# happyjin/Gaussian_process

Hardware: AMD Instinct MI355X
Metric: GP-fit+predict sec and achieved fp64 TFLOP/s, N=65536 d=8, 1/2/4/8 MI355X (higher is better)
Workload: dtype f64; 1 GPU; GP fit+predict N=65536 d=8 n_test=4096 (BASELINE configs[2]); N=65536, d=8, n_test=4096, partition=single GPU

## Files before the change

### gaussian_process_amd/csrc/dev_api.hip

```cpp
#include "gpmi_ctx.h"

using namespace gpmi;

extern "C" {

int gpmi_dev_rbf_rows(void* stream, const double* X_dev, int64_t N, int64_t d, int64_t row0,
                      int64_t nrows, int64_t ncols, double sigma, double ell, double noise_var,
                      double* out_dev, int64_t ld) {
    if (!X_dev || !out_dev) return fail_arg("gpmi_dev_rbf_rows: null pointer");
    if (nrows % TILE || ncols % TILE || row0 % TILE || ld < ncols || ld % 2)
        return fail_arg("gpmi_dev_rbf_rows: sizes must be multiples of 128");
    RbfArgs r;
    r.A = r.B = X_dev; r.nA = r.nB = N; r.d = d; r.row0 = row0; r.nrows = nrows; r.ncols = ncols;
    r.coef = -.5 * (1 / (ell * ell)); r.sig2 = sigma * sigma; r.diag_add = noise_var; r.symmetric = 1;
    r.out = out_dev; r.ld = ld;
    HIP_TRY(launch_rbf((hipStream_t)stream, r));
    return GPMI_OK;
}

int gpmi_dev_rbf_cross(void* stream, const double* Xs_dev, int64_t n, const double* X_dev, int64_t N,
                       int64_t d, int64_t row0, int64_t nrows, int64_t ncols, double sigma, double ell,
                       double* out_dev, int64_t ld) {
    if (!Xs_dev || !X_dev || !out_dev) return fail_arg("gpmi_dev_rbf_cross: null pointer");
    if (nrows % TILE || ncols % TILE || ld < ncols || ld % 2)
// ... 48 lines not shown
                       int64_t ncols, double* out_dev, int64_t ld) {
    if (!Xs_dev || !Xcols_dev || !out_dev) return fail_arg("gpmi_dev_cov_cross: null pointer");
    if (nrows % TILE || ncols % TILE || ld < ncols || ld % 2 || col0 < 0)
        return fail_arg("gpmi_dev_cov_cross: sizes must be multiples of 128");
    RbfArgs r;
    r.A = Xs_dev; r.B = Xcols_dev; r.nA = n; r.nB = ncols_real > 0 ? ncols_real : 0; r.d = d; r.row0 = 0; r.nrows = nrows; r.ncols = ncols;
    const int rc = dev_cov_args(r, kind, params, nparams, "gpmi_dev_cov_cross");
    if (rc) return rc;
    r.diag_add = 0.; r.symmetric = 0; r.delta_square = square ? 1 : 0; r.delta_col0 = col0;
    r.out = out_dev; r.ld = ld;
    HIP_TRY(launch_rbf((hipStream_t)stream, r));
    return GPMI_OK;
}

int gpmi_dev_potrf_block(void* stream, double* A_dev, int64_t ld, int64_t nb, int64_t col_offset,
                         int64_t* info_dev) {
    if (!A_dev || !info_dev) return fail_arg("gpmi_dev_potrf_block: null pointer");
    if (nb <= 0 || nb % TILE || ld % 2) return fail_arg("gpmi_dev_potrf_block: nb must be a multiple of 128");
    HIP_TRY(panel_factor((hipStream_t)stream, A_dev, ld, nb, nb, col_offset, info_dev));
    return GPMI_OK;
}

int gpmi_dev_trsm_block(void* stream, const double* L_dev, int64_t ldl, double* X_dev, int64_t ldx,
                        int64_t m, int64_t nb) {
    if (!L_dev || !X_dev) return fail_arg("gpmi_dev_trsm_block: null pointer");
    if (m < 0 || m % TILE || nb <= 0 || nb % IB || ldl % 2 || ldx % 2)
        return fail_arg("gpmi_dev_trsm_block: m must be a multiple of 128, nb of 64");
    if (m == 0) return GPMI_OK;
    HIP_TRY(trsm_block((hipStream_t)stream, L_dev, ldl, X_dev, ldx, m, nb));
    return GPMI_OK;
}

int gpmi_dev_border_sweep(void* stream, const double* L_dev, int64_t ldl, int64_t ncols, double* X_dev, int64_t ldx,
                          int64_t rows) {
    if (!L_dev || !X_dev) return fail_arg("gpmi_dev_border_sweep: null pointer");
    if (rows < 1 || rows > 16) return fail_arg("gpmi_dev_border_sweep: rows must be in 1..16");
    if (ncols < 0 || ncols % TILE) return fail_arg("gpmi_dev_border_sweep: ncols must be a multiple of 128");
    if (ldl % 2 || ldx % 2 || ldl < ncols || ldx < ncols)
        return fail_arg("gpmi_dev_border_sweep: ldl and ldx must be even and at least ncols");
    if ((reinterpret_cast<uintptr_t>(L_dev) & 15) || (reinterpret_cast<uintptr_t>(X_dev) & 15))
        return fail_arg("gpmi_dev_border_sweep: both pointers must be 16-byte aligned");
    HIP_TRY(launch_border_sweep((hipStream_t)stream, L_dev, ldl, ncols, X_dev, ldx, rows));
    return GPMI_OK;
}

int gpmi_dev_gemm_nt(void* stream, double* C_dev, int64_t ldc, const double* A_dev, int64_t lda,
                     const double* B_dev, int64_t ldb, int64_t M, int64_t N, int64_t K, int lower,
                     int64_t diag_off) {
    if (!C_dev || !A_dev || !B_dev) return fail_arg("gpmi_dev_gemm_nt: null pointer");
    if (M < 0 || N < 0 || K < 0 || M % TILE || N % IB || K % 16 || ldc % 2 || lda % 2 || ldb % 2)
        return fail_arg("gpmi_dev_gemm_nt: M%128, N%64, K%16 must be 0");
    GemmArgs g = gemm_minus(C_dev, ldc, A_dev, lda, B_dev, ldb, M, N, K);
    g.lower = lower; g.diag_off = diag_off;
    HIP_TRY(launch_gemm_nt((hipStream_t)stream, g));
    return GPMI_OK;
}

int gpmi_dev_gemm_nt_rowmap(void* stream, double* C_dev, int64_t ldc, const double* A_dev, int64_t lda,
                            const double* B_dev, int64_t ldb, int64_t M, int64_t N, int64_t K,
                            const int32_t* row_ncols_dev, int64_t row_block_rows) {
    if (!C_dev || !A_dev || !B_dev || !row_ncols_dev) return fail_arg("gpmi_dev_gemm_nt_rowmap: null pointer");
    if (M < 0 || N < 0 || K < 0 || M % TILE || N % IB || K % 16 || ldc % 2 || lda % 2 || ldb % 2 ||
        row_block_rows <= 0 || row_block_rows % TILE)
        return fail_arg("gpmi_dev_gemm_nt_rowmap: M%128, N%64, K%16, row_block_rows%128 must be 0");
    GemmArgs g = gemm_minus(C_dev, ldc, A_dev, lda, B_dev, ldb, M, N, K);
    g.row_ncols = row_ncols_dev; g.row_block_tiles = (int)(row_block_rows / TILE);
    HIP_TRY(launch_gemm_nt((hipStream_t)stream, g));
    return GPMI_OK;
}

int gpmi_dev_gemm_nt_rowmap_host(void* stream, double* C_dev, int64_t ldc, const double* A_dev, int64_t lda,
                                 const double* B_dev, int64_t ldb, int64_t M, int64_t N, int64_t K,
                                 const int32_t* row_ncols_dev, const int32_t* row_ncols_host, int64_t row_bands,
                                 int64_t row_block_rows) {
    if (!C_dev || !A_dev || !B_dev || !row_ncols_dev || !row_ncols_host) return fail_arg("gpmi_dev_gemm_nt_rowmap_host: null pointer");
    if (M < 0 || N < 0 || K < 0 || M % TILE || N % IB || K % 16 || ldc % 2 || lda % 2 || ldb % 2 ||
        row_block_rows <= 0 || row_block_rows % TILE || row_bands * row_block_rows < M)
        return fail_arg("gpmi_dev_gemm_nt_rowmap_host: M%128, N%64, K%16, row_block_rows%128 must be 0 and the map must cover M");
    GemmArgs g = gemm_minus(C_dev, ldc, A_dev, lda, B_dev, ldb, M, N, K);
    g.row_ncols = row_ncols_dev; g.row_block_tiles = (int)(row_block_rows / TILE);
    g.row_ncols_host = row_ncols_host; g.row_bands = (int)row_bands;
    HIP_TRY(launch_gemm_nt((hipStream_t)stream, g));
    return GPMI_OK;
}

int gpmi_dev_gemm_nt_blocks(void* stream, double* C_dev, int64_t ldc, const double* A_dev, int64_t lda,
                            const double* B_dev, int64_t ldb, const int64_t* b_block_off_dev, int64_t b_block_rows,
                            int64_t M, int64_t N, int64_t K, const int32_t* row_ncols_dev,
                            const int32_t* row_ncols_host, int64_t row_bands, int64_t row_block_rows) {
    if (!C_dev || !A_dev || !B_dev || !b_block_off_dev) return fail_arg("gpmi_dev_gemm_nt_blocks: null pointer");
    if (M < 0 || N < 0 || K < 0 || M % TILE || N % TILE || K % 16 || K < 32 || ldc % 2 || lda % 2 || ldb % 2 ||
        b_block_rows <= 0 || b_block_rows % TILE)
        return fail_arg("gpmi_dev_gemm_nt_blocks: M%128, N%128, K%16 (K >= 32), b_block_rows%128 must be 0");
    if ((row_ncols_dev != nullptr) != (row_ncols_host != nullptr))
        return fail_arg("gpmi_dev_gemm_nt_blocks: the row map needs both its device and its host copy");
    if (row_ncols_dev && (row_block_rows <= 0 || row_block_rows % TILE || row_bands * row_block_rows < M))
        return fail_arg("gpmi_dev_gemm_nt_blocks: row_block_rows%128 must be 0 and the map must cover M");
    GemmArgs g = gemm_minus(C_dev, ldc, A_dev, lda, B_dev, ldb, M, N, K);
    g.b_block_off = b_block_off_dev; g.b_block_rows = b_block_rows;
    if (row_ncols_dev) {
        g.row_ncols = row_ncols_dev; g.row_block_tiles = (int)(row_block_rows / TILE);
        g.row_ncols_host = row_ncols_host; g.row_bands = (int)row_bands;
    }
    HIP_TRY(launch_gemm_nt((hipStream_t)stream, g));
    return GPMI_OK;
}
// ... 104 lines not shown
```

### gaussian_process_amd/csrc/driver.hip

```cpp
#include "gpmi_ctx.h"
#include "gpmi_plan.h"

namespace gpmi {

hipError_t panel_rec(hipStream_t s, double* A, int64_t ld, int64_t mrows, int64_t off, int64_t w,
                     int64_t col_offset, int64_t* info) {
    hipError_t e;
    const bool fused = tuning().panel_fused && w % 128 == 0 && off % 128 == 0;
    const int64_t leaf = fused ? 128 : IB;
    if (w <= leaf) {
        double* Ajj = A + off * ld + off;
        const int64_t below = mrows - off - leaf;
        if (fused) {
            if ((e = launch_potrf128(s, Ajj, ld, col_offset + off, info)) != hipSuccess) return e;
            if (below > 0) return launch_trsm128(s, Ajj, ld, A + (off + leaf) * ld + off, ld, below);
            return hipSuccess;
        }
        if ((e = launch_potf2_64(s, Ajj, ld, col_offset + off, info)) != hipSuccess) return e;
        if (below > 0) return launch_trsm_rlt64(s, Ajj, ld, A + (off + IB) * ld + off, ld, below);
        return hipSuccess;
    }
    const int64_t h = (w / 2) / leaf * leaf;
    if ((e = panel_rec(s, A, ld, mrows, off, h, col_offset, info)) != hipSuccess) return e;
    {
        const int64_t c0 = off + h;
        const int64_t r0 = c0 / TILE * TILE;
        const GemmArgs g = gemm_minus_lower(A + r0 * ld + c0, ld, A + r0 * ld + off, ld, A + c0 * ld + off, ld, mrows - r0,
                                            w - h, h, r0 - c0);
        if ((e = launch_gemm_nt(s, g)) != hipSuccess) return e;
    }
    return panel_rec(s, A, ld, mrows, off + h, w - h, col_offset, info);
}

hipError_t panel_factor(hipStream_t s, double* A, int64_t ld, int64_t nb, int64_t mrows,
                        int64_t col_offset, int64_t* info) {
    return panel_rec(s, A, ld, mrows, 0, nb, col_offset, info);
}

hipError_t trsm_rec(hipStream_t s, const double* L, int64_t ldl, double* X, int64_t ldx, int64_t m,
                    int64_t off, int64_t w) {
    hipError_t e;
    const bool fused = tuning().panel_fused && w % 128 == 0 && off % 128 == 0 && m % 128 == 0;
    const int64_t leaf = fused ? 128 : IB;
    if (w <= leaf) {
        if (fused) return launch_trsm128(s, L + off * ldl + off, ldl, X + off, ldx, m);
        return launch_trsm_rlt64(s, L + off * ldl + off, ldl, X + off, ldx, m);
    }
    const int64_t h = (w / 2) / leaf * leaf;
    if ((e = trsm_rec(s, L, ldl, X, ldx, m, off, h)) != hipSuccess) return e;
    const GemmArgs g = gemm_minus(X + off + h, ldx, X + off, ldx, L + (off + h) * ldl + off, ldl, m, w - h, h);
    if ((e = launch_gemm_nt(s, g)) != hipSuccess) return e;
    return trsm_rec(s, L, ldl, X, ldx, m, off + h, w - h);
}

hipError_t trsm_block(hipStream_t s, const double* L, int64_t ldl, double* X, int64_t ldx,
                      int64_t m, int64_t nb) {
    return trsm_rec(s, L, ldl, X, ldx, m, 0, nb);
}

hipError_t cholesky_inplace(gpmi_ctx* c, double* A, int64_t ld, int64_t ncols, int64_t nrows,
                            int64_t* info, bool account, int64_t carried_rows) {
    hipError_t e;
    hipStream_t sm = c->stream;
    const int64_t NB = c->block(ncols);
    const bool la = c->lookahead_for(ncols);
    hipStream_t sp_ = la ? c->pstream : sm;
    const bool slack = la && ncols >= 49152;
    SharingScope shallow(la ? Sharing::beside_update().with_panel_slack(slack) : sharing());
    const int slot_p = account ? GPMI_T_CHOL_PANEL : GPMI_T_COUNT - 1;
    const int slot_t = account ? GPMI_T_CHOL_TRAIL : GPMI_T_COUNT - 1;
    if (la && (e = c->order(sm, sp_)) != hipSuccess) return e;
    auto trail = [&](hipStream_t st, bool counted, int64_t r0, int64_t c0, int64_t k, int64_t nb, int64_t ncol_upd) -> hipError_t {
        GemmArgs g = gemm_minus_lower(A + r0 * ld + c0, ld, A + r0 * ld + k, ld, A + c0 * ld + k, ld, nrows - r0, ncol_upd,
                                      nb, r0 - c0);
        g.role = counted ? 1 : 0;
        const GemmRoute route = gemm_nt_route(g);
        const bool dma = gemm_kernel_is_dma(route.kernel);
        size_t sp = c->span_begin(counted ? (dma ? slot_t : GPMI_T_COUNT - 1) : slot_p, st);
        hipError_t er = launch_gemm_nt(st, g, route);
        c->span_end(sp, st);
        if (account && dma && counted) {
            c->stage_ms[GPMI_T_TRAIL_LAUNCHES] += 1.0;
            c->stage_ms[GPMI_T_TRAIL_FLOPS] += gemm_nt_algorithmic_flops(g, ncols - r0 + 1 + carried_rows);
        }
        return er;
    };
    hipEvent_t ev_b = nullptr;
    for (int64_t k = 0; k < ncols; k += NB) {
        const int64_t nb = std::min<int64_t>(NB, ncols - k);
        size_t sp = c->span_begin(slot_p, sp_);
        {
            SharingScope panel_forms(!la ? sharing().large_lds()
                                     : (ncols - k >= c->shallow_min ? Sharing::beside_update() : Sharing::chip_shared_only()).with_panel_slack(slack));
            e = panel_factor(sp_, A + k * ld + k, ld, nb, nrows - k, k, info);
        }
        c->span_end(sp, sp_);
        if (e != hipSuccess) return e;
        if (la && (e = c->order(sp_, sm)) != hipSuccess) return e;
        const int64_t r0 = k + nb;
        if (r0 >= ncols) continue;
        if (!la) {
            if ((e = trail(sm, true, r0, r0, k, nb, ncols - r0)) != hipSuccess) return e;
            continue;
        }
        const int64_t nbn = std::min<int64_t>(NB, ncols - r0);
        if (ev_b && (e = hipStreamWaitEvent(sp_, ev_b, 0)) != hipSuccess) return e;
        if ((e = trail(sp_, false, r0, r0, k, nb, nbn)) != hipSuccess) return e;
        if (r0 + nbn < ncols) {
            if ((e = trail(sm, true, r0 + nbn, r0 + nbn, k, nb, ncols - r0 - nbn)) != hipSuccess) return e;
            ev_b = c->new_event();
            if (!ev_b) return c->ev_error;
            if ((e = hipEventRecord(ev_b, sm)) != hipSuccess) return e;
        }
    }
    return hipSuccess;
}

RbfArgs rbf_cross(const gpmi_ctx* c, const double* A, int64_t nA, const Box& ba, const double* B, int64_t nB, const Box& bb,
                  int64_t row0, int64_t nrows, int64_t ncols, double* out, int64_t ld) {
    RbfArgs r;
    r.A = A; r.B = B;
    r.nA = nA; r.nB = nB; r.d = c->d; r.row0 = row0; r.nrows = nrows; r.ncols = ncols;
    r.coef = c->coef; r.sig2 = c->sig2;
    r.kind = c->kind; r.kp0 = c->kp0; r.kp1 = c->kp1;
    for (int i = 0; i < 11; ++i) r.kpv[i] = c->kpv[i];
    r.diag_add = 0.; r.symmetric = 0;
    r.delta_square = (A == c->x_test() && B == c->x_train() && nA == nB) ? 1 : 0;
    r.max_sq = box_max_sq(ba, bb);
// ... 202 lines not shown
```

### gaussian_process_amd/csrc/gemm_dma.hip

```cpp
#include <algorithm>
#include <cstdlib>
#include <type_traits>

#include "gpmi_internal.h"
#include "gpmi_plan.h"
#include <atomic>
#include <mutex>

namespace gpmi {

typedef double d4 __attribute__((ext_vector_type(4)));
typedef double d2 __attribute__((ext_vector_type(2)));

#define GPMI_LDS __attribute__((address_space(3)))
#define GPMI_GLB __attribute__((address_space(1)))
#define GPMI_CONST __attribute__((address_space(4)))

struct GemmDmaDev {
    double* C;
    const double* A;
    const double* B;
    int64_t ldc, lda, ldb;
    int Tm, Tn;
    int nchunks;
    int lower;
    int64_t diag_off;
    const int32_t* row_ncols;
    int row_block_tiles;
    const int64_t* b_block_off;
    int b_block_tiles;
    int S, logS, SM, SN, tri, nsuper;
    int pair;
    int sprefix[DMA_MAX_SM + 1];
    unsigned long long* stamps;
    int dbg;
    struct PersistSlot* slot;
    int nblocks;
};

struct PersistSlot {
    unsigned ctr[8];
    unsigned done;
    unsigned pad[7];
};

template <class PT>
__device__ __forceinline__ bool dma_block_to_tile(const PT& p, int b, int& ti, int& tj) {
    return plan_block_to_tile(p, b, ti, tj);
}

__device__ __forceinline__ bool dma_map_tile(const GemmDmaDev& p, int& ti, int& tj) {
    return dma_block_to_tile(p, blockIdx.x, ti, tj);
}

constexpr int DMA_TM = PLAN_TILE, DMA_TN = PLAN_TILE;
template <class PT>
__device__ __forceinline__ bool dma_tile_live(const PT& p, int ti, int tj) {
    return plan_tile_live(p, ti, tj, p.row_ncols);
}
constexpr int DMA_STAGE_SLOTS = (DMA_TM + DMA_TN) * 8;
constexpr int DMA_STAGES = 3;

constexpr unsigned TICKET_NONE = 0xFFFFFFFFu;

template <class PT>
__device__ __forceinline__ unsigned ticket_draw(const PT& p, int xcd) {
    const unsigned per = (unsigned)p.nblocks >> 3;
#pragma unroll 1
    for (int t = 0; t < 8; ++t) {
        const int x = (xcd + t) & 7;
        if (t && __hip_atomic_load(&p.slot->ctr[x], __ATOMIC_RELAXED, __HIP_MEMORY_SCOPE_AGENT) >= per) continue;
        const unsigned w = atomicAdd(&p.slot->ctr[x], 1u);
        if (w < per) return w * 8u + (unsigned)x;
    }
    return TICKET_NONE;
}

template <int MI, bool DBG, bool TICKET = false>
__device__ __forceinline__ void gemm_nt_dma_body(const GemmDmaDev& p) {
    constexpr int NWAVES = 16 / MI;
    constexpr int DPW = 32 / NWAVES;
    constexpr int RPW = DMA_TM / NWAVES;
    constexpr int NFR = MI + 4;
    const int dbg = DBG ? p.dbg : 0;
    extern __shared__ __attribute__((aligned(16))) char smem_raw[];
    const int tid = threadIdx.x;
    volatile GPMI_LDS int* mbox = (volatile GPMI_LDS int*)(smem_raw + DMA_STAGES * DMA_STAGE_SLOTS * 16);
    unsigned blk = blockIdx.x, nxt_blk = TICKET_NONE;
    int par = 0;
    if constexpr (TICKET) {
        if (tid == 0) mbox[0] = (int)ticket_draw(p, (int)(blockIdx.x & 7));
        __syncthreads();
        blk = (unsigned)__builtin_amdgcn_readfirstlane(mbox[0]);
        par = 1;
    }
  for (;;) {
    int ti = 0, tj = 0;
    bool live;
    if constexpr (TICKET) {
        if (blk == TICKET_NONE) break;
// ... 793 lines not shown
hipError_t launch_gemm_nt_small(hipStream_t s, const GemmArgs& a, const GemmRoute& r) {
    GemmSmallDev p;
    p.C = a.C; p.A = a.A; p.B = a.B; p.ldc = a.ldc; p.lda = a.lda; p.ldb = a.ldb;
    p.Tm = (int)(a.M / SM_T); p.Tn = (int)(a.N / SM_T); p.nchunks = (int)(a.K / 16);
    p.lower = a.lower; p.diag_off = a.diag_off;
    static PerDeviceOnce once;
    const hipError_t ea = once.run([&]() -> hipError_t {
        return hipFuncSetAttribute((const void*)gemm_nt_small_kernel<8>, hipFuncAttributeMaxDynamicSharedMemorySize, (int)(8 * GEMM_SMALL_STAGE));
    });
    if (ea != hipSuccess) return ea;
    if (r.kernel == GemmKernel::Small3) hipLaunchKernelGGL(gemm_nt_small_kernel<3>, dim3(r.grid), dim3(256), r.lds, s, p);
    else hipLaunchKernelGGL(gemm_nt_small_kernel<8>, dim3(r.grid), dim3(256), r.lds, s, p);
    return hipGetLastError();
}

struct PersistPool {
    static constexpr int SLOTS = 16384;
    PersistSlot* base = nullptr;
    int groups = 0;
    std::atomic<unsigned> head{0};
    PersistSlot* next() { return base + (head.fetch_add(1, std::memory_order_relaxed) % SLOTS); }
};

static PersistPool* persist_pool() {
    static std::mutex mu;
    static PersistPool pools[16];
    int dev = 0;
    if (hipGetDevice(&dev) != hipSuccess || dev < 0 || dev >= 16) return nullptr;
    PersistPool& pl = pools[dev];
    std::lock_guard<std::mutex> lock(mu);
    if (!pl.base) {
        hipDeviceProp_t prop;
        if (hipGetDeviceProperties(&prop, dev) != hipSuccess) return nullptr;
        void* q = nullptr;
        if (hipMalloc(&q, sizeof(PersistSlot) * PersistPool::SLOTS) != hipSuccess) return nullptr;
        if (hipMemset(q, 0, sizeof(PersistSlot) * PersistPool::SLOTS) != hipSuccess) { (void)hipFree(q); return nullptr; }
        pl.groups = (prop.multiProcessorCount / 8) * 8;
        if (pl.groups < 8) { (void)hipFree(q); return nullptr; }
        const void* fns[] = {(const void*)gemm_nt_dma_persist_kernel, (const void*)chol_trailing_update_persist_kernel,
                             (const void*)gemm_nt_dma_ticket_kernel, (const void*)chol_trailing_update_ticket_kernel};
        for (const void* f : fns)
            if (hipFuncSetAttribute(f, hipFuncAttributeMaxDynamicSharedMemorySize,
                                    (int)(DMA_STAGES * DMA_STAGE_SLOTS * 16 + 16)) != hipSuccess) { (void)hipFree(q); return nullptr; }
        pl.base = static_cast<PersistSlot*>(q);
    }
    return &pl;
}

int gemm_resident_groups() {
    const PersistPool* pool = persist_pool();
    return pool ? pool->groups : 0;
}

static_assert((size_t)DMA_STAGES * DMA_STAGE_SLOTS * 16 == GEMM_DMA_LDS && TALL_LDS == GEMM_TALL_LDS && TALL_LDS == GEMM_DMA_LDS,
              "gpmi_route.h sizes the rings of the launches; one opt-in size serves both forms");

hipError_t launch_gemm_nt_dma(hipStream_t s, const GemmArgs& a, const GemmRoute& r) {
    const TilePlan& plan = r.plan;
    GemmDmaDev p;
    p.C = a.C; p.A = a.A; p.B = a.B;
    p.ldc = a.ldc; p.lda = a.lda; p.ldb = a.ldb;
    p.Tm = plan.Tm; p.Tn = plan.Tn;
    p.nchunks = (int)(a.K / 16);
    p.lower = a.lower; p.diag_off = a.diag_off;
    p.row_ncols = a.row_ncols; p.row_block_tiles = plan.row_block_tiles;
    p.b_block_off = a.b_block_off;
    p.b_block_tiles = a.b_block_off ? (int)(a.b_block_rows / 128) : 1;
    p.S = plan.S; p.logS = plan.logS; p.SM = plan.SM; p.SN = plan.SN; p.tri = plan.tri; p.nsuper = plan.nsuper;
    p.pair = plan.pair;
    if (plan.tri == 2) std::copy(plan.sprefix, plan.sprefix + plan.SM + 1, p.sprefix);
    p.dbg = tuning().gemm_dbg & 0xff;
    p.stamps = tuning().gemm_stamps;
    p.slot = nullptr;
    p.nblocks = plan.nblocks;
    static PerDeviceOnce once;
    const hipError_t ea = once.run([&]() -> hipError_t {
        const void* fns[] = {(const void*)gemm_nt_dma_kernel<4, false>, (const void*)gemm_nt_dma_kernel<4, true>,
                             (const void*)gemm_nt_dma_kernel<2, false>, (const void*)gemm_nt_dma_kernel<2, true>,
                             (const void*)chol_trailing_update_dma_kernel, (const void*)gemm_nt_dma_tall_kernel<false>,
                             (const void*)gemm_nt_dma_tall_kernel<true>, (const void*)chol_trailing_update_dma256_kernel};
        for (const void* f : fns) {
            const hipError_t e = hipFuncSetAttribute(f, hipFuncAttributeMaxDynamicSharedMemorySize, (int)GEMM_DMA_LDS);
            if (e != hipSuccess) return e;
        }
        return hipSuccess;
    });
    if (ea != hipSuccess) return ea;
    if (r.kernel >= GemmKernel::Persist) {
        PersistPool* pool = persist_pool();
        if (!pool) return hipErrorInvalidValue;
        p.slot = pool->next();
    }
    const dim3 grid(r.grid);
    switch (r.kernel) {
        case GemmKernel::Ticket: hipLaunchKernelGGL(gemm_nt_dma_ticket_kernel, grid, dim3(512), r.lds, s, p); break;
        case GemmKernel::TicketTrail: hipLaunchKernelGGL(chol_trailing_update_ticket_kernel, grid, dim3(512), r.lds, s, p); break;
        case GemmKernel::Persist: hipLaunchKernelGGL(gemm_nt_dma_persist_kernel, grid, dim3(512), r.lds, s, p); break;
        case GemmKernel::PersistTrail: hipLaunchKernelGGL(chol_trailing_update_persist_kernel, grid, dim3(512), r.lds, s, p); break;
        case GemmKernel::Tall: hipLaunchKernelGGL(gemm_nt_dma_tall_kernel<false>, grid, dim3(512), r.lds, s, p); break;
        case GemmKernel::TallProbe: hipLaunchKernelGGL(gemm_nt_dma_tall_kernel<true>, grid, dim3(512), r.lds, s, p); break;
        case GemmKernel::TallTrail: hipLaunchKernelGGL(chol_trailing_update_dma256_kernel, grid, dim3(512), r.lds, s, p); break;
        case GemmKernel::Dma8: hipLaunchKernelGGL((gemm_nt_dma_kernel<2, false>), grid, dim3(512), r.lds, s, p); break;
        case GemmKernel::Dma8Probe: hipLaunchKernelGGL((gemm_nt_dma_kernel<2, true>), grid, dim3(512), r.lds, s, p); break;
        case GemmKernel::Dma8Trail: hipLaunchKernelGGL(chol_trailing_update_dma_kernel, grid, dim3(512), r.lds, s, p); break;
        case GemmKernel::Dma4: hipLaunchKernelGGL((gemm_nt_dma_kernel<4, false>), grid, dim3(256), r.lds, s, p); break;
        case GemmKernel::Dma4Probe: hipLaunchKernelGGL((gemm_nt_dma_kernel<4, true>), grid, dim3(256), r.lds, s, p); break;
        default: return hipErrorInvalidValue;
    }
    return hipGetLastError();
}

}
```

### gaussian_process_amd/csrc/gpmi_api.hip

```cpp
#include "gpmi_ctx.h"

using namespace gpmi;

namespace gpmi {
thread_local std::string g_err;

static thread_local Tuning t_dev_tuning;
static thread_local const Tuning* t_tuning = nullptr;
const Tuning& tuning() { return t_tuning ? *t_tuning : t_dev_tuning; }
TuneScope::TuneScope(const Tuning* t) : prev(t_tuning) { t_tuning = t; }
TuneScope::~TuneScope() { t_tuning = prev; }
static thread_local Sharing t_sharing;
Sharing& sharing() { return t_sharing; }

int ard_rescale_train(gpmi_ctx* c) {
    if (!c->ard()) return GPMI_OK;
    HIP_TRY(c->Xz.ensure((size_t)c->N * c->d * 8));
    HIP_TRY(launch_scale_inputs(c->stream, c->X.as<double>(), c->ard_rdev.as<double>(), c->N, c->d, c->Xz.as<double>()));
    HIP_TRY(hipStreamSynchronize(c->stream));
    box_scale(c->boxX, c->ard_r, c->boxZ);
    return GPMI_OK;
}
int ard_rescale_test(gpmi_ctx* c) {
    if (!c->ard()) return GPMI_OK;
    HIP_TRY(c->Xsz.ensure((size_t)c->n * c->d * 8));
    HIP_TRY(launch_scale_inputs(c->stream, c->Xs.as<double>(), c->ard_rdev.as<double>(), c->n, c->d, c->Xsz.as<double>()));
    HIP_TRY(hipStreamSynchronize(c->stream));
    box_scale(c->boxXs, c->ard_r, c->boxZs);
    return GPMI_OK;
}
}

extern "C" {

int gpmi_abi_version(void) { return GPMI_ABI_VERSION; }
const char* gpmi_last_error(void) { return g_err.c_str(); }

int gpmi_device_count(int* count) {
    if (!count) return fail_arg("gpmi_device_count: null pointer");
    int n = 0;
    hipError_t e = hipGetDeviceCount(&n);
    if (e != hipSuccess) { *count = 0; return fail_runtime(e, "hipGetDeviceCount"); }
    *count = n;
    return GPMI_OK;
}

int gpmi_ctx_create(int device, gpmi_ctx** out) {
    if (!out) return fail_arg("gpmi_ctx_create: null out pointer");
    *out = nullptr;
    int n = 0;
    HIP_TRY(hipGetDeviceCount(&n));
    if (device < 0 || device >= n) return fail_arg("gpmi_ctx_create: no such device");
    HIP_TRY(hipSetDevice(device));
    gpmi_ctx* c = new gpmi_ctx();
    c->device = device;
    int prio_lo = 0, prio_hi = 0;
    (void)hipDeviceGetStreamPriorityRange(&prio_lo, &prio_hi);
    hipError_t e = hipStreamCreateWithPriority(&c->stream, hipStreamNonBlocking, prio_lo);
    if (e != hipSuccess) { delete c; return fail_runtime(e, "hipStreamCreate"); }
    e = hipStreamCreateWithPriority(&c->pstream, hipStreamNonBlocking, prio_hi);
    if (e != hipSuccess) { (void)hipStreamDestroy(c->stream); delete c; return fail_runtime(e, "hipStreamCreate"); }
    const char* env;
    if ((env = getenv("GPMI_NB"))) c->nb = std::max<int64_t>(128, atoll(env) / 128 * 128);
    if ((env = getenv("GPMI_LD_PAD"))) c->ld_pad = std::max<int64_t>(0, atoll(env) / 2 * 2);
    if ((env = getenv("GPMI_LOOKAHEAD"))) c->lookahead = atoi(env) ? 1 : 0;
    *out = c;
    return GPMI_OK;
}

int gpmi_ctx_destroy(gpmi_ctx* c) {
    if (!c) return GPMI_OK;
    for (gpmi_ctx* l : c->lane_ctx) (void)gpmi_ctx_destroy(l);
    c->lane_ctx.clear();
    (void)hipSetDevice(c->device);
    (void)hipStreamSynchronize(c->stream);
    for (DevBuf* b : {&c->X, &c->y, &c->A, &c->info, &c->red, &c->Xs, &c->V, &c->P, &c->vec, &c->dense,
                       &c->U, &c->Kn, &c->gpart, &c->cov_a, &c->cov_b, &c->cov_out, &c->flag, &c->vside,
                       &c->Xz, &c->Xsz, &c->ard_rdev, &c->gsum, &c->app, &c->lap, &c->lap_part, &c->lap_out, &c->sm, &c->sm_part, &c->sm_E, &c->sm_B, &c->sm_out, &c->loov, &c->loow,
                       &c->sp_Zraw, &c->sp_Z, &c->sp_L, &c->sp_B, &c->sp_W, &c->sp_q, &c->sp_vec, &c->sp_part, &c->sp_scr, &c->sp_info, &c->sp_pred,
                       &c->sp_g0, &c->sp_g1, &c->sp_g2, &c->sp_gE, &c->sp_gpart, &c->sp_gvec})
        b->release();
    for (auto e : c->ev_pool) (void)hipEventDestroy(e);
    (void)hipStreamDestroy(c->stream);
    (void)hipStreamDestroy(c->pstream);
    delete c;
    return GPMI_OK;
}

static int set_tuning_option(Tuning& t, const char* name, int64_t value) {
    if (!strcmp(name, "gemm_small_tiles")) {
        t.gemm_small_tiles = value ? 1 : 0;
    } else if (!strcmp(name, "trsm_wave")) {
        t.trsm_wave = value ? 1 : 0;
    } else if (!strcmp(name, "gemm_small_dma")) {
        t.gemm_small_dma = value ? 1 : 0;
    } else if (!strcmp(name, "gemm_persist")) {
        t.gemm_persist = value ? 1 : 0;
    } else if (!strcmp(name, "gemm_ticket")) {
        if (value < 0 || value > 2) return fail_arg("gemm_ticket must be 0 (off), 1 (trailing updates under lookahead) or 2 (every launch)");
        t.gemm_ticket = (int)value;
    } else if (!strcmp(name, "gemm_balance")) {
        t.gemm_balance = value ? 1 : 0;
    } else if (!strcmp(name, "trsv_vinv")) {
        if (value < 0 || value > 2) return fail_arg("trsv_vinv must be 0 (16 x 16 rounds), 1 (one launch per block) or 2 (one launch)");
        t.trsv_vinv = (int)value;
    } else if (!strcmp(name, "panel_fused")) {
        t.panel_fused = value ? 1 : 0;
    } else if (!strcmp(name, "rbf_blocks")) {
        if (value < 1 || value > (1 << 24)) return fail_arg("rbf_blocks must be in 1..2^24");
        t.rbf_blocks = (int)value;
    } else if (!strcmp(name, "gemm_dma_waves")) {
        if (value != 4 && value != 8) return fail_arg("gemm_dma_waves must be 4 or 8");
        t.gemm_dma_waves = (int)value;
    } else if (!strcmp(name, "gemm_tall")) {
        if (value < 0 || value > 1) return fail_arg("gemm_tall must be 0 (128 x 128 blocks) or 1 (256 x 128 blocks for large launches)");
        t.gemm_tall = (int)value;
    } else if (!strcmp(name, "tall_min_tiles")) {
        if (value < 0 || value > (1 << 30)) return fail_arg("tall_min_tiles must be in 0..2^30");
        t.tall_min_tiles = (int)value;
    } else if (!strcmp(name, "tall_min_tiles_slack")) {
        if (value < 0 || value > (1 << 30)) return fail_arg("tall_min_tiles_slack must be in 0..2^30");
        t.tall_min_tiles_slack = (int)value;
    } else if (!strcmp(name, "gemm_dma")) {
        t.gemm_use_dma = value ? 1 : 0;
    } else {
        return -1;
    }
    return GPMI_OK;
}

int gpmi_set_option(gpmi_ctx* c, const char* name, int64_t value) {
    if (!c || !name) return fail_arg("gpmi_set_option: null argument");
    if (!strcmp(name, "nb")) {
        if (value != 0 && (value < 128 || value % 128)) return fail_arg("nb must be 0 (auto) or a positive multiple of 128");
        c->nb = value;
    } else if (!strcmp(name, "ld_pad")) {
        if (value < 0 || value % 2) return fail_arg("ld_pad must be even and >= 0");
        c->ld_pad = value;
        c->res.drop_fit();
    } else if (!strcmp(name, "timing")) {
        c->timing = value ? 1 : 0;
    } else if (!strcmp(name, "lookahead")) {
        c->lookahead = value ? 1 : 0;
    } else if (!strcmp(name, "la_min")) {
        if (value < 0) return fail_arg("la_min must be >= 0");
        c->la_min = value;
    } else if (!strcmp(name, "shallow_min")) {
        if (value < 0) return fail_arg("shallow_min must be >= 0");
        c->shallow_min = value;
    } else if (!strcmp(name, "sparse_slab")) {
        if (value < 0) return fail_arg("sparse_slab must be >= 0 (0: by size)");
        c->sparse_slab = value;
    } else if (!strcmp(name, "reserve")) {
        if (value < 0) return fail_arg("reserve must be >= 0 (points that gpmi_append may add in place)");
        c->reserve = value;
    } else if (!strcmp(name, "append_skinny")) {
        if (value < -1 || value > 1) return fail_arg("append_skinny must be -1 (by size), 0 (never) or 1 (whenever allowed)");
        c->append_skinny = (int)value;
    } else if (!strcmp(name, "lanes")) {
        if (value < 0 || value > 8) return fail_arg("lanes must be 0 (by size) .. 8");
        c->lanes = (int)value;
    } else {
        const int rc = set_tuning_option(c->tune, name, value);
        if (rc < 0) return fail_arg("gpmi_set_option: unknown option");
        return rc;
    }
    return GPMI_OK;
}

int gpmi_dev_set_option(const char* name, int64_t value) {
    if (!name) return fail_arg("gpmi_dev_set_option: null argument");
    const int rc = set_tuning_option(t_dev_tuning, name, value);
    if (rc < 0) return fail_arg("gpmi_dev_set_option: unknown option");
    return rc;
}

int gpmi_set_kernel(gpmi_ctx* c, int kind, double p0, double p1) {
// ... 295 lines not shown
    HIP_TRY(hipSetDevice(c->device));
    const Tuning tn = resident_tuning(c);
    TuneScope tune_scope(&tn);
    return lml_grad_ard_impl(c, d_r, d_ell, d_sigma, d_noise);
}

int gpmi_lml_grad_co2(gpmi_ctx* c, double* d_theta, double* d_noise) {
    if (!c) return fail_arg("gpmi_lml_grad_co2: null context");
    HIP_TRY(hipSetDevice(c->device));
    const Tuning tn = resident_tuning(c);
    TuneScope tune_scope(&tn);
    return lml_grad_co2_impl(c, d_theta, d_noise);
}

int gpmi_loo(gpmi_ctx* c, double* mu, double* var, double* logp, double* loo) {
    if (!c) return fail_arg("gpmi_loo: null context");
    HIP_TRY(hipSetDevice(c->device));
    const Tuning tn = resident_tuning(c);
    TuneScope tune_scope(&tn);
    return loo_impl(c, mu, var, logp, loo);
}

int gpmi_loo_grad(gpmi_ctx* c, double* d_ell, double* d_sigma, double* d_noise) {
    if (!c) return fail_arg("gpmi_loo_grad: null context");
    HIP_TRY(hipSetDevice(c->device));
    const Tuning tn = resident_tuning(c);
    TuneScope tune_scope(&tn);
    return loo_grad_impl(c, d_ell, d_sigma, d_noise);
}

int gpmi_grad_trace(gpmi_ctx* c, const double* a_in, const double* b_in, int64_t N, int64_t d, double sigma,
                    double ell, const double* alpha_in, const double* Kinv_in, double* d_ell, double* d_sigma) {
    if (!c || !a_in || !b_in || !alpha_in || !Kinv_in || !d_ell || !d_sigma) return fail_arg("gpmi_grad_trace: null argument");
    HIP_TRY(hipSetDevice(c->device));
    return grad_trace_impl(c, a_in, b_in, N, d, sigma, ell, alpha_in, Kinv_in, d_ell, d_sigma);
}

int gpmi_post_chol(gpmi_ctx* c, double jitter, double* L_out, int64_t* bad_pivot) {
    if (!c || !L_out) return fail_arg("gpmi_post_chol: null argument");
    HIP_TRY(hipSetDevice(c->device));
    TuneScope tune_scope(&c->tune);
    return post_chol_impl(c, jitter, L_out, bad_pivot);
}

int gpmi_post_sample(gpmi_ctx* c, double jitter, const double* Z, int64_t num_fun, double* LZ_out, int64_t* bad_pivot) {
    if (!c || !Z || !LZ_out) return fail_arg("gpmi_post_sample: null argument");
    HIP_TRY(hipSetDevice(c->device));
    TuneScope tune_scope(&c->tune);
    return post_sample_impl(c, jitter, Z, num_fun, LZ_out, bad_pivot);
}

static int lane_prepare(gpmi_ctx* c, gpmi_ctx* l) {
    l->nb = c->nb; l->ld_pad = c->ld_pad; l->lookahead = c->lookahead; l->la_min = c->la_min; l->timing = c->timing;
    l->tune = c->tune;
    l->kind = c->kind; l->kp0 = c->kp0; l->kp1 = c->kp1;
    for (int i = 0; i < 11; ++i) l->kpv[i] = c->kpv[i];
    l->N = c->N; l->d = c->d; l->boxX = c->box_train();
    HIP_TRY(l->X.ensure((size_t)c->N * c->d * 8));
    HIP_TRY(l->y.ensure((size_t)c->N * 8));
    HIP_TRY(hipMemcpyAsync(l->X.p, c->x_train(), (size_t)c->N * c->d * 8, hipMemcpyDeviceToDevice, l->stream));
    HIP_TRY(hipMemcpyAsync(l->y.p, c->y.p, (size_t)c->N * 8, hipMemcpyDeviceToDevice, l->stream));
    HIP_TRY(hipStreamSynchronize(l->stream));
    l->res.drop_train();
    l->res.train_set();
    return GPMI_OK;
}

int gpmi_lml_batch(gpmi_ctx* c, const double* triples, int64_t T, double* lml_out, int* status_out) {
    if (!c || !triples || !lml_out) return fail_arg("gpmi_lml_batch: null argument");
    if (T < 0) return fail_arg("gpmi_lml_batch: T < 0");
    if (!c->res.have_train) return fail_arg("gpmi_lml_batch: no training set (call gpmi_set_train)");
    HIP_TRY(hipSetDevice(c->device));
    const int64_t Np = round_up(c->N, TILE);
    int L = c->lanes ? c->lanes : (Np > 32768 ? 1 : Np >= 24576 ? 3 : Np >= 12288 ? 5 : 4);
    L = (int)std::min<int64_t>(L, std::max<int64_t>(T, 1));
    struct LaMinScope {
        gpmi_ctx* c; int64_t keep;
        ~LaMinScope() { c->la_min = keep; }
    } la_scope{c, c->la_min};
    if (L > 1) c->la_min = std::max<int64_t>(c->la_min, 12288);
    while ((int)c->lane_ctx.size() < L - 1) {
        gpmi_ctx* l = nullptr;
        int rc = gpmi_ctx_create(c->device, &l);
        if (rc) return rc;
        c->lane_ctx.push_back(l);
    }
    for (int j = 0; j < L - 1; ++j) {
        int rc = lane_prepare(c, c->lane_ctx[(size_t)j]);
        if (rc) return rc;
    }
    const int parent_class = (int)((T - 1 + L) % L);
    std::vector<gpmi_ctx*> lane((size_t)L);
    for (int r = 0, nx = 0; r < L; ++r) lane[(size_t)r] = (r == parent_class) ? c : c->lane_ctx[(size_t)nx++];
    std::vector<int> lane_rc((size_t)L, GPMI_OK);
    std::vector<std::string> lane_err((size_t)L);
    std::vector<std::vector<double>> lane_ms((size_t)L, std::vector<double>(GPMI_T_COUNT, 0.0));
    auto work = [&](int r) {
        gpmi_ctx* l = lane[(size_t)r];
        TuneScope tune_scope(&l->tune);
        SharingScope shares_chip(L > 1 ? sharing().and_chip_shared() : sharing());
        if (hipSetDevice(l->device) != hipSuccess) { lane_rc[(size_t)r] = GPMI_ERR_RUNTIME; lane_err[(size_t)r] = "hipSetDevice"; return; }
        for (int64_t t = r; t < T; t += L) {
            const double ell = triples[3 * t], sigma = triples[3 * t + 1], s2 = triples[3 * t + 2];
            double lml = 0.;
            int64_t bad = 0;
            const int rc = factorize_impl(l, sigma, ell, s2, &lml, &bad);
            if (rc == GPMI_ERR_RUNTIME || rc == GPMI_ERR_BAD_ARG) {
// ... 103 lines not shown
```

### gaussian_process_amd/csrc/gpmi_internal.h

```cpp
#pragma once
#include <hip/hip_runtime.h>
#include <stdint.h>

#include <cmath>
#include <mutex>

#include "gpmi_kroute.h"
#include "gpmi_route.h"

namespace gpmi {

constexpr int TILE = 128;
constexpr int IB = 64;

struct Tuning : GemmTuning {
    int trsm_wave = 1;
    int rbf_blocks = 16384;
    int trsv_vinv = 2;
    int panel_fused = 1;
    unsigned long long* gemm_stamps = nullptr;
    unsigned long long* panel_stamps = nullptr;
};
const Tuning& tuning();
struct TuneScope {
    const Tuning* prev;
    explicit TuneScope(const Tuning* t);
    ~TuneScope();
};
Sharing& sharing();
struct SharingScope {
    const Sharing prev;
    explicit SharingScope(Sharing s) : prev(sharing()) { sharing() = s; }
    ~SharingScope() { sharing() = prev; }
};

struct PerDeviceOnce {
    std::mutex mu;
    uint64_t done = 0;
    template <class F> hipError_t run(F fn) {
        int dev = 0;
        hipError_t e = hipGetDevice(&dev);
        if (e != hipSuccess) return e;
        std::lock_guard<std::mutex> lock(mu);
        if (dev < 64 && ((done >> dev) & 1)) return hipSuccess;
        e = fn();
        if (e == hipSuccess && dev < 64) done |= (uint64_t)1 << dev;
        return e;
    }
};

struct GemmArgs {
    double* C;
    const double* A;
    const double* B;
    int64_t ldc, lda, ldb;
    int64_t M, N, K;
    int mode = 0;
    int lower = 0;
    int64_t diag_off = 0;
    const int32_t* row_ncols = nullptr;
    int row_block_tiles = 1;
    const int32_t* row_ncols_host = nullptr;
    int row_bands = 0;
    int role = 0;
    const int64_t* b_block_off = nullptr;
    int64_t b_block_rows = 0;
};
inline GemmArgs gemm_minus(double* C, int64_t ldc, const double* A, int64_t lda, const double* B, int64_t ldb, int64_t M,
                           int64_t N, int64_t K) {
    GemmArgs g;
    g.C = C; g.A = A; g.B = B;
    g.ldc = ldc; g.lda = lda; g.ldb = ldb;
    g.M = M; g.N = N; g.K = K;
    return g;
}
inline GemmArgs gemm_minus_lower(double* C, int64_t ldc, const double* A, int64_t lda, const double* B, int64_t ldb,
                                 int64_t M, int64_t N, int64_t K, int64_t diag_off) {
    GemmArgs g = gemm_minus(C, ldc, A, lda, B, ldb, M, N, K);
    g.lower = 1; g.diag_off = diag_off;
    return g;
}
GemmRoute gemm_nt_route(const GemmArgs& a);
hipError_t launch_gemm_nt(hipStream_t s, const GemmArgs& a, const GemmRoute& r);
inline hipError_t launch_gemm_nt(hipStream_t s, const GemmArgs& a) { return launch_gemm_nt(s, a, gemm_nt_route(a)); }
double gemm_nt_algorithmic_flops(const GemmArgs& a, int64_t real_rows);
hipError_t launch_gemm_nt_dma(hipStream_t s, const GemmArgs& a, const GemmRoute& r);
hipError_t launch_gemm_nt_small(hipStream_t s, const GemmArgs& a, const GemmRoute& r);
int gemm_resident_groups();
double gemm_nt_flops(const GemmArgs& a);

hipError_t launch_potf2_64(hipStream_t s, double* A, int64_t ld, int64_t col_offset,
                           int64_t* info_dev);
hipError_t launch_trsm_rlt64(hipStream_t s, const double* L, int64_t ldl, double* X, int64_t ldx,
                             int64_t m);

hipError_t launch_potrf128(hipStream_t s, double* A, int64_t ld, int64_t col_offset, int64_t* info_dev);

hipError_t launch_trsm128(hipStream_t s, const double* L, int64_t ldl, double* X, int64_t ldx, int64_t m);

hipError_t launch_border_sweep(hipStream_t s, const double* L, int64_t ldl, int64_t ncols, double* X, int64_t ldx,
                               int64_t rows);

struct RbfArgs {
    const double* A;
    const double* B;
    int64_t nA, nB, d;
    int64_t row0;
    int64_t nrows;
    int64_t ncols;
    double coef;
    double sig2;
    double diag_add;
    int symmetric;
    double* out;
    int64_t ld;
    int kind = 0;
    double kp0 = 0., kp1 = 0.;
// ... 114 lines not shown
```

### gaussian_process_amd/csrc/gpmi_plan.h

```cpp
#pragma once
#include <math.h>
#include <stdint.h>

#include <algorithm>

#if defined(__HIPCC__)
#define GPMI_HD __host__ __device__ __forceinline__
#else
#define GPMI_HD inline
#endif

namespace gpmi {

constexpr int PLAN_TILE = 128;
constexpr int DMA_MAX_SM = 128;

struct TilePlan {
    int Tm = 0, Tn = 0;
    int lower = 0;
    int64_t diag_off = 0;
    int row_block_tiles = 1;
    int S = 1, logS = 0, SM = 0, SN = 0;
    int tri = 0;
    int nsuper = 0;
    int nblocks = 0;
    int pair = 0;
    int sprefix[DMA_MAX_SM + 1];
    const int32_t* row_ncols = nullptr;
};

template <class PT>
GPMI_HD bool plan_block_to_tile(const PT& p, int b, int& ti, int& tj) {
    const int xcd = b & 7;
    const int w = b >> 3;
    const int S2 = (p.S * p.S) >> p.pair;
    const int s = (w / S2) * 8 + xcd;
    if (s >= p.nsuper) return false;
    const int q = w % S2;
    int si, sj;
    if (p.tri == 2) {
        si = 0;
        while (si + 1 < p.SM && p.sprefix[si + 1] <= s) ++si;
        sj = s - p.sprefix[si];
        if (sj == p.sprefix[si + 1] - p.sprefix[si] - 1 && p.row_ncols) {
            int acc = 0;
            for (int r = 0; r < (p.S >> p.pair); ++r) {
                const int tr = si * p.S + (r << p.pair);
                int w = 0;
                for (int h = 0; h <= p.pair; ++h) {
                    if (tr + h >= p.Tm) break;
                    const int64_t nc = p.row_ncols[(tr + h) / p.row_block_tiles];
                    int64_t wl = (nc + PLAN_TILE - 1) / PLAN_TILE - (int64_t)sj * p.S;
                    if (wl > p.S) wl = p.S;
                    if (wl > (int64_t)p.Tn - (int64_t)sj * p.S) wl = (int64_t)p.Tn - (int64_t)sj * p.S;
                    if (wl > w) w = (int)wl;
                }
                if (q < acc + w) {
// ... 95 lines not shown
    while (S > 1 && (S > p.Tn || S > p.Tm)) S >>= 1;
    const int min_S = pair ? 2 : 1;
    if (S < min_S) S = min_S;
    if (force_S && force_S < min_S) return false;
    if (!force_S && balance_xcds && S > 2 &&
        ((p.tri == 1 && !stairs && p.Tn <= 256) || (stairs && (int64_t)p.Tm * p.Tn <= 32768))) {
        double eff[4] = {0., 0., 0., 0.}, best = 0.0;
        int cand[4], nc = 0;
        for (int c = S; c >= 2 && nc < 4; c >>= 1) {
            TilePlan q;
            if (!plan_tiles(q, Tm, Tn, lower, diag_off, has_row_map, row_ncols_host, row_bands, row_block_tiles, c, false, pair)) break;
            if (stairs && q.tri != 2) break;
            cand[nc] = c;
            eff[nc] = plan_xcd_efficiency(q, row_ncols_host);
            best = std::max(best, eff[nc]);
            ++nc;
        }
        for (int i = 0; i < nc; ++i)
            if (eff[i] >= best - 0.01) { force_S = cand[i]; break; }
    }
    if (force_S) S = force_S;
    for (;; S >>= 1) {
        const int SM = (p.Tm + S - 1) / S, SN = (p.Tn + S - 1) / S;
        int ns = p.tri ? SM * (SM + 1) / 2 : SM * SN;
        bool use_stairs = false;
        if (stairs && SM <= DMA_MAX_SM) {
            int tot = 0;
            p.sprefix[0] = 0;
            for (int si = 0; si < SM; ++si) {
                int64_t widest = 0;
                for (int ti = si * S; ti < std::min((si + 1) * S, p.Tm); ++ti) {
                    const int band = std::min(ti / p.row_block_tiles, row_bands - 1);
                    widest = std::max<int64_t>(widest, row_ncols_host[band]);
                }
                widest = std::max<int64_t>(widest, 0);
                const int64_t live = std::min<int64_t>(SN, (widest + (int64_t)S * PLAN_TILE - 1) / ((int64_t)S * PLAN_TILE));
                tot += (int)live;
                p.sprefix[si + 1] = tot;
            }
            ns = tot;
            use_stairs = true;
        }
        if (ns >= 32 || S == min_S || force_S) {
            p.S = S; p.SM = SM; p.SN = SN; p.nsuper = ns;
            if (use_stairs) { p.tri = 2; p.row_ncols = row_ncols_host; }
            break;
        }
    }
    p.logS = (p.S == 8) ? 3 : (p.S == 4) ? 2 : (p.S == 2) ? 1 : 0;
    p.nblocks = ((p.nsuper + 7) / 8) * 8 * ((p.S * p.S) >> p.pair);
    return true;
}

inline int64_t plan_live_tiles(int64_t Tm, int64_t Tn, int lower, int64_t diag_off, const int32_t* row_ncols_host,
                               int row_bands, int row_block_tiles) {
    int64_t n = 0;
    const int rbt = row_block_tiles > 0 ? row_block_tiles : 1;
    for (int64_t ti = 0; ti < Tm; ++ti) {
        int64_t w = Tn;
        if (lower) {
            const int64_t lim = ti * PLAN_TILE + PLAN_TILE - 1 + diag_off;
            w = lim < 0 ? 0 : std::min<int64_t>(Tn, lim / PLAN_TILE + 1);
        }
        if (row_ncols_host && row_bands > 0) {
            const int64_t nc = row_ncols_host[std::min<int64_t>(ti / rbt, row_bands - 1)];
            w = std::min<int64_t>(w, nc > 0 ? (nc + PLAN_TILE - 1) / PLAN_TILE : 0);
        }
        n += w;
    }
    return n;
}

inline double plan_tile_flops(int64_t M, int64_t N, int64_t K, int lower, int64_t diag_off) {
    if (M <= 0 || N <= 0 || K <= 0) return 0.;
    const int TN = (N % 128 == 0) ? 128 : 64;
    const int64_t Tm = M / 128, Tn = N / TN;
    int64_t tiles = 0;
    for (int64_t ti = 0; ti < Tm; ++ti) {
        if (!lower) { tiles += Tn; continue; }
        const int64_t lim = ti * 128 + 127 + diag_off;
        if (lim < 0) continue;
        const int64_t cnt = lim / TN + 1;
        tiles += cnt < Tn ? cnt : Tn;
    }
    return 2.0 * (double)tiles * 128.0 * TN * (double)K;
}

inline double plan_algorithmic_flops(int64_t M, int64_t N, int64_t K, int lower, int64_t diag_off, int64_t real_rows) {
    if (M <= 0 || N <= 0 || K <= 0) return 0.;
    const int64_t rows = std::min<int64_t>(M, real_rows);
    if (!lower) return 2.0 * (double)rows * (double)N * (double)K;
    double elems = 0.;
    const int64_t r_full = std::max<int64_t>(0, N - 1 - diag_off);
    const int64_t r_first = std::max<int64_t>(0, -diag_off);
    const int64_t tri_end = std::min(rows, r_full);
    if (tri_end > r_first) {
        const double n = (double)(tri_end - r_first);
        const double first = (double)(r_first + diag_off + 1);
        elems += n * first + n * (n - 1) / 2.0;
    }
    if (rows > r_full) elems += (double)(rows - std::max(r_full, (int64_t)0)) * (double)N;
    return 2.0 * elems * (double)K;
}

}
```

Measured before the change: 69.40 TFLOP/s.

## Add precomputed per-XCD balanced block tables for tall DMA GEMM updates

Builds a host-side table that maps grid blocks to live tiles for the tall DMA GEMM kernels. Supertiles are greedily balanced across the 8 XCDs using cost weights (full vs half-live pairs), and the table is cached on the device per plan shape. Trailing and panel updates opt in via a dense_grid flag, so the launch grid shrinks to the compacted table size. The aim is to remove dead blocks and XCD load imbalance in the triangular updates, at the cost of a table lookup per block plus a one-time allocation and copy for each new plan shape.

```diff
diff --git a/gaussian_process_amd/csrc/dev_api.hip b/gaussian_process_amd/csrc/dev_api.hip
--- a/gaussian_process_amd/csrc/dev_api.hip
+++ b/gaussian_process_amd/csrc/dev_api.hip
@@ -124,6 +124,7 @@
         return fail_arg("gpmi_dev_gemm_nt: M%128, N%64, K%16 must be 0");
     GemmArgs g = gemm_minus(C_dev, ldc, A_dev, lda, B_dev, ldb, M, N, K);
     g.lower = lower; g.diag_off = diag_off;
+    g.dense_grid = sharing().panel_slack;
     HIP_TRY(launch_gemm_nt((hipStream_t)stream, g));
     return GPMI_OK;
 }
diff --git a/gaussian_process_amd/csrc/driver.hip b/gaussian_process_amd/csrc/driver.hip
--- a/gaussian_process_amd/csrc/driver.hip
+++ b/gaussian_process_amd/csrc/driver.hip
@@ -25,8 +25,9 @@
     {
         const int64_t c0 = off + h;
         const int64_t r0 = c0 / TILE * TILE;
-        const GemmArgs g = gemm_minus_lower(A + r0 * ld + c0, ld, A + r0 * ld + off, ld, A + c0 * ld + off, ld, mrows - r0,
-                                            w - h, h, r0 - c0);
+        GemmArgs g = gemm_minus_lower(A + r0 * ld + c0, ld, A + r0 * ld + off, ld, A + c0 * ld + off, ld, mrows - r0, w - h, h,
+                                      r0 - c0);
+        g.dense_grid = true;
         if ((e = launch_gemm_nt(s, g)) != hipSuccess) return e;
     }
     return panel_rec(s, A, ld, mrows, off + h, w - h, col_offset, info);
@@ -74,6 +75,7 @@
         GemmArgs g = gemm_minus_lower(A + r0 * ld + c0, ld, A + r0 * ld + k, ld, A + c0 * ld + k, ld, nrows - r0, ncol_upd,
                                       nb, r0 - c0);
         g.role = counted ? 1 : 0;
+        g.dense_grid = true;
         const GemmRoute route = gemm_nt_route(g);
         const bool dma = gemm_kernel_is_dma(route.kernel);
         size_t sp = c->span_begin(counted ? (dma ? slot_t : GPMI_T_COUNT - 1) : slot_p, st);
diff --git a/gaussian_process_amd/csrc/gemm_dma.hip b/gaussian_process_amd/csrc/gemm_dma.hip
--- a/gaussian_process_amd/csrc/gemm_dma.hip
+++ b/gaussian_process_amd/csrc/gemm_dma.hip
@@ -36,6 +36,7 @@
     int dbg;
     struct PersistSlot* slot;
     int nblocks;
+    const uint32_t* block_table;
 };
 
 struct PersistSlot {
@@ -46,6 +47,12 @@
 
 template <class PT>
 __device__ __forceinline__ bool dma_block_to_tile(const PT& p, int b, int& ti, int& tj) {
+    if (p.block_table) {
+        const uint32_t e = p.block_table[b];
+        ti = (int)(e >> 16);
+        tj = (int)(e & 0xffffu);
+        return e != PLAN_TABLE_PAD;
+    }
     return plan_block_to_tile(p, b, ti, tj);
 }
 
@@ -945,6 +952,38 @@
     return pool ? pool->groups : 0;
 }
 
+const BlockTables::Entry* BlockTables::get(const TilePlan& plan, hipError_t* err) {
+    *err = hipSuccess;
+    int dev = 0;
+    if ((*err = hipGetDevice(&dev)) != hipSuccess) return nullptr;
+    for (const Entry& e : entries)
+        if (e.device == dev && e.Tm == plan.Tm && e.Tn == plan.Tn && e.lower == plan.lower && e.diag_off == plan.diag_off &&
+            e.S == plan.S && e.tri == plan.tri && e.nsuper == plan.nsuper)
+            return e.dev ? &e : nullptr;
+    if (entries.size() >= MAX_TABLES) return nullptr;
+    const std::vector<uint32_t> t = plan_block_table(plan, nullptr);
+    Entry e{dev, plan.Tm, plan.Tn, plan.lower, plan.S, plan.tri, plan.nsuper, plan.diag_off, nullptr, (unsigned)t.size()};
+    if (!t.empty() && bytes + t.size() * sizeof(uint32_t) <= MAX_BYTES) {
+        void* q = nullptr;
+        if ((*err = hipMalloc(&q, t.size() * sizeof(uint32_t))) != hipSuccess) return nullptr;
+        if ((*err = hipMemcpy(q, t.data(), t.size() * sizeof(uint32_t), hipMemcpyHostToDevice)) != hipSuccess) {
+            (void)hipFree(q);
+            return nullptr;
+        }
+        e.dev = static_cast<uint32_t*>(q);
+        bytes += t.size() * sizeof(uint32_t);
+    }
+    entries.push_back(e);
+    return e.dev ? &entries.back() : nullptr;
+}
+
+void BlockTables::release() {
+    for (Entry& e : entries)
+        if (e.dev) (void)hipFree(e.dev);
+    entries.clear();
+    bytes = 0;
+}
+
 static_assert((size_t)DMA_STAGES * DMA_STAGE_SLOTS * 16 == GEMM_DMA_LDS && TALL_LDS == GEMM_TALL_LDS && TALL_LDS == GEMM_DMA_LDS,
               "gpmi_route.h sizes the rings of the launches; one opt-in size serves both forms");
 
@@ -966,6 +1005,15 @@
     p.stamps = tuning().gemm_stamps;
     p.slot = nullptr;
     p.nblocks = plan.nblocks;
+    p.block_table = nullptr;
+    unsigned nblocks = r.grid;
+    if (a.dense_grid && (r.kernel == GemmKernel::Tall || r.kernel == GemmKernel::TallTrail) && !a.row_ncols && plan.tri != 2 &&
+        tuning().update_table && tuning().tables) {
+        hipError_t et;
+        const BlockTables::Entry* t = tuning().tables->get(plan, &et);
+        if (et != hipSuccess) return et;
+        if (t) { p.block_table = t->dev; nblocks = t->grid; }
+    }
     static PerDeviceOnce once;
     const hipError_t ea = once.run([&]() -> hipError_t {
         const void* fns[] = {(const void*)gemm_nt_dma_kernel<4, false>, (const void*)gemm_nt_dma_kernel<4, true>,
@@ -984,7 +1032,7 @@
         if (!pool) return hipErrorInvalidValue;
         p.slot = pool->next();
     }
-    const dim3 grid(r.grid);
+    const dim3 grid(nblocks);
     switch (r.kernel) {
         case GemmKernel::Ticket: hipLaunchKernelGGL(gemm_nt_dma_ticket_kernel, grid, dim3(512), r.lds, s, p); break;
         case GemmKernel::TicketTrail: hipLaunchKernelGGL(chol_trailing_update_ticket_kernel, grid, dim3(512), r.lds, s, p); break;
diff --git a/gaussian_process_amd/csrc/gpmi_api.hip b/gaussian_process_amd/csrc/gpmi_api.hip
--- a/gaussian_process_amd/csrc/gpmi_api.hip
+++ b/gaussian_process_amd/csrc/gpmi_api.hip
@@ -7,7 +7,11 @@
 
 static thread_local Tuning t_dev_tuning;
 static thread_local const Tuning* t_tuning = nullptr;
-const Tuning& tuning() { return t_tuning ? *t_tuning : t_dev_tuning; }
+const Tuning& tuning() {
+    if (t_tuning) return *t_tuning;
+    if (!t_dev_tuning.tables) t_dev_tuning.tables = new BlockTables();
+    return t_dev_tuning;
+}
 TuneScope::TuneScope(const Tuning* t) : prev(t_tuning) { t_tuning = t; }
 TuneScope::~TuneScope() { t_tuning = prev; }
 static thread_local Sharing t_sharing;
@@ -64,6 +68,8 @@
     if ((env = getenv("GPMI_NB"))) c->nb = std::max<int64_t>(128, atoll(env) / 128 * 128);
     if ((env = getenv("GPMI_LD_PAD"))) c->ld_pad = std::max<int64_t>(0, atoll(env) / 2 * 2);
     if ((env = getenv("GPMI_LOOKAHEAD"))) c->lookahead = atoi(env) ? 1 : 0;
+    if ((env = getenv("GPMI_UPDATE_TABLE"))) c->tune.update_table = atoi(env) ? 1 : 0;
+    c->tune.tables = new BlockTables();
     *out = c;
     return GPMI_OK;
 }
@@ -80,6 +86,8 @@
                        &c->sp_Zraw, &c->sp_Z, &c->sp_L, &c->sp_B, &c->sp_W, &c->sp_q, &c->sp_vec, &c->sp_part, &c->sp_scr, &c->sp_info, &c->sp_pred,
                        &c->sp_g0, &c->sp_g1, &c->sp_g2, &c->sp_gE, &c->sp_gpart, &c->sp_gvec})
         b->release();
+    delete c->tune.tables;
+    c->tune.tables = nullptr;
     for (auto e : c->ev_pool) (void)hipEventDestroy(e);
     (void)hipStreamDestroy(c->stream);
     (void)hipStreamDestroy(c->pstream);
@@ -123,6 +131,8 @@
         t.tall_min_tiles_slack = (int)value;
     } else if (!strcmp(name, "gemm_dma")) {
         t.gemm_use_dma = value ? 1 : 0;
+    } else if (!strcmp(name, "update_table")) {
+        t.update_table = value ? 1 : 0;
     } else {
         return -1;
     }
@@ -524,7 +534,9 @@
 
 static int lane_prepare(gpmi_ctx* c, gpmi_ctx* l) {
     l->nb = c->nb; l->ld_pad = c->ld_pad; l->lookahead = c->lookahead; l->la_min = c->la_min; l->timing = c->timing;
+    BlockTables* own = l->tune.tables;
     l->tune = c->tune;
+    l->tune.tables = own;
     l->kind = c->kind; l->kp0 = c->kp0; l->kp1 = c->kp1;
     for (int i = 0; i < 11; ++i) l->kpv[i] = c->kpv[i];
     l->N = c->N; l->d = c->d; l->boxX = c->box_train();
diff --git a/gaussian_process_amd/csrc/gpmi_internal.h b/gaussian_process_amd/csrc/gpmi_internal.h
--- a/gaussian_process_amd/csrc/gpmi_internal.h
+++ b/gaussian_process_amd/csrc/gpmi_internal.h
@@ -4,6 +4,7 @@
 
 #include <cmath>
 #include <mutex>
+#include <vector>
 
 #include "gpmi_kroute.h"
 #include "gpmi_route.h"
@@ -13,7 +14,24 @@
 constexpr int TILE = 128;
 constexpr int IB = 64;
 
+struct BlockTables {
+    struct Entry {
+        int device, Tm, Tn, lower, S, tri, nsuper;
+        int64_t diag_off;
+        uint32_t* dev;
+        unsigned grid;
+    };
+    static constexpr size_t MAX_TABLES = 512, MAX_BYTES = (size_t)64 << 20;
+    std::vector<Entry> entries;
+    size_t bytes = 0;
+    const Entry* get(const TilePlan& plan, hipError_t* err);
+    void release();
+    ~BlockTables() { release(); }
+};
+
 struct Tuning : GemmTuning {
+    int update_table = 1;
+    BlockTables* tables = nullptr;
     int trsm_wave = 1;
     int rbf_blocks = 16384;
     int trsv_vinv = 2;
@@ -63,6 +81,7 @@
     const int32_t* row_ncols_host = nullptr;
     int row_bands = 0;
     int role = 0;
+    bool dense_grid = false;
     const int64_t* b_block_off = nullptr;
     int64_t b_block_rows = 0;
 };
diff --git a/gaussian_process_amd/csrc/gpmi_plan.h b/gaussian_process_amd/csrc/gpmi_plan.h
--- a/gaussian_process_amd/csrc/gpmi_plan.h
+++ b/gaussian_process_amd/csrc/gpmi_plan.h
@@ -3,6 +3,7 @@
 #include <stdint.h>
 
 #include <algorithm>
+#include <vector>
 
 #if defined(__HIPCC__)
 #define GPMI_HD __host__ __device__ __forceinline__
@@ -204,6 +205,87 @@
     return true;
 }
 
+constexpr uint32_t PLAN_TABLE_PAD = 0xFFFFFFFFu;
+constexpr double PLAN_HALF_BLOCK_COST = 0.53;
+struct BlockCosts {
+    double full = 1.0;
+    double half = PLAN_HALF_BLOCK_COST;
+};
+
+inline std::vector<uint32_t> plan_block_table(const TilePlan& p, const int32_t* row_ncols_host, BlockCosts costs = BlockCosts()) {
+    std::vector<uint32_t> table;
+    if (!p.pair || p.Tm > 65535 || p.Tn > 65535 || p.nsuper <= 0) return table;
+    struct Item { uint32_t e; double c; };
+    const int S2 = (p.S * p.S) >> p.pair;
+    std::vector<std::vector<Item>> super((size_t)p.nsuper);
+    std::vector<double> scost((size_t)p.nsuper, 0.0);
+    for (int b = 0; b < p.nblocks; ++b) {
+        int ti, tj;
+        if (!plan_block_to_tile(p, b, ti, tj)) continue;
+        bool l0, l1;
+        plan_pair_live(p, ti, tj, row_ncols_host, l0, l1);
+        if (!l0 && !l1) continue;
+        const int s = ((b >> 3) / S2) * 8 + (b & 7);
+        const double c = (l0 && l1) ? costs.full : costs.half;
+        super[(size_t)s].push_back(Item{((uint32_t)ti << 16) | (uint32_t)tj, c});
+        scost[(size_t)s] += c;
+    }
+    std::vector<int> order((size_t)p.nsuper);
+    for (int s = 0; s < p.nsuper; ++s) order[(size_t)s] = s;
+    std::stable_sort(order.begin(), order.end(), [&](int a, int b) { return scost[(size_t)a] > scost[(size_t)b]; });
+    std::vector<Item> xcd[8];
+    double xc[8] = {0., 0., 0., 0., 0., 0., 0., 0.};
+    auto cheapest = [&]() { int k = 0; for (int x = 1; x < 8; ++x) if (xc[x] < xc[k]) k = x; return k; };
+    auto dearest = [&]() { int k = 0; for (int x = 1; x < 8; ++x) if (xc[x] > xc[k]) k = x; return k; };
+    size_t total = 0;
+    for (int s : order) {
+        if (super[(size_t)s].empty()) continue;
+        const int k = cheapest();
+        xcd[k].insert(xcd[k].end(), super[(size_t)s].begin(), super[(size_t)s].end());
+        xc[k] += scost[(size_t)s];
+        total += super[(size_t)s].size();
+    }
+    for (size_t moves = 0; moves < 8 * total; ++moves) {
+        const int hi = dearest(), lo = cheapest();
+        if (!(xc[hi] - xc[lo] > costs.full) || xcd[hi].empty()) break;
+        const Item it = xcd[hi].back();
+        if (!(it.c > 0.0) || !(it.c < xc[hi] - xc[lo])) break;
+        xcd[hi].pop_back();
+        xcd[lo].push_back(it);
+        xc[hi] -= it.c;
+        xc[lo] += it.c;
+    }
+    size_t len = 0;
+    for (int x = 0; x < 8; ++x) {
+        std::stable_sort(xcd[x].begin(), xcd[x].end(), [](const Item& a, const Item& b) { return a.c > b.c; });
+        len = std::max(len, xcd[x].size());
+    }
+    table.assign(8 * len, PLAN_TABLE_PAD);
+    for (int x = 0; x < 8; ++x)
+        for (size_t j = 0; j < xcd[x].size(); ++j) table[8 * j + (size_t)x] = xcd[x][j].e;
+    return table;
+}
+
+inline long plan_paid_slots(const TilePlan& p, const int32_t* row_ncols_host, const std::vector<uint32_t>* table) {
+    long load[32];
+    for (int x = 0; x < 32; ++x) load[x] = 0;
+    if (table) {
+        for (size_t b = 0; b < table->size(); ++b)
+            if ((*table)[b] != PLAN_TABLE_PAD) ++load[b & 31];
+    } else {
+        for (int b = 0; b < p.nblocks; ++b) {
+            int ti, tj;
+            if (!plan_block_to_tile(p, b, ti, tj)) continue;
+            bool l0, l1;
+            plan_pair_live(p, ti, tj, row_ncols_host, l0, l1);
+            if (l0 || l1) ++load[b & 31];
+        }
+    }
+    long rounds = 0;
+    for (int x = 0; x < 32; ++x) rounds = std::max(rounds, (load[x] + 7) / 8);
+    return rounds * 512;
+}
+
 inline int64_t plan_live_tiles(int64_t Tm, int64_t Tn, int lower, int64_t diag_off, const int32_t* row_ncols_host,
                                int row_bands, int row_block_tiles) {
     int64_t n = 0;
```

After: 69.88 TFLOP/s, median of 6. About the same (+0.7%).
